# xyfJASON/ctrlora

Hardware: NVIDIA H100
Metric: ddim_steps_per_sec (higher is better)
Workload: dtype fp16 (fp32 accumulate)

## Files before the change

ctrlora_b200/csrc/gemm_sm90.cu:

```cuda
#include "gemm_sm90.cuh"
#include "wgmma.cuh"
#include "ctrlora_b200.h"
#include <stdio.h>
#include <string.h>

namespace ctrl {

__device__ __forceinline__ bool aligned16(const void* ptr) { return (reinterpret_cast<uintptr_t>(ptr) & 15) == 0; }
__device__ __forceinline__ uint32_t pack_h2(float a, float b) {
    __half2 h = __floats2half2_rn(a, b);
    return *reinterpret_cast<uint32_t*>(&h);
}

template <int CW>
__device__ __forceinline__ void epilogue_chunk(const GemmKParams& p, float* v, int c, int bn_out, int n0, bool row_ok,
                                               long long m, int img, int tok) {
    const int nbase = n0 + c;
    const bool full_chunk = (c + CW <= bn_out) && (nbase + CW <= p.N);
    if (!row_ok) return;
    if (p.rowbias) {
        const float* rb = p.rowbias + static_cast<long long>(img) * p.rowbias_ld + nbase;
        if (full_chunk && aligned16(rb)) {
#pragma unroll
            for (int q = 0; q < CW / 4; ++q) {
                const float4 b4 = __ldg(reinterpret_cast<const float4*>(rb) + q);
                v[4 * q] += b4.x; v[4 * q + 1] += b4.y; v[4 * q + 2] += b4.z; v[4 * q + 3] += b4.w;
            }
        } else {
#pragma unroll
            for (int j = 0; j < CW; ++j)
                if (nbase + j < p.N) v[j] += __ldg(rb + j);
        }
    }
    if (p.out_scale != 1.0f) {
#pragma unroll
        for (int j = 0; j < CW; ++j) v[j] *= p.out_scale;
    }
    if (p.residual && p.residual_f32) {
        const float* rp = reinterpret_cast<const float*>(p.residual) + m * p.ldr + nbase;
        if (full_chunk && aligned16(rp)) {
#pragma unroll
            for (int q = 0; q < CW / 4; ++q) {
                const float4 r4 = __ldg(reinterpret_cast<const float4*>(rp) + q);
                v[4 * q] += r4.x; v[4 * q + 1] += r4.y; v[4 * q + 2] += r4.z; v[4 * q + 3] += r4.w;
            }
        } else {
#pragma unroll
            for (int j = 0; j < CW; ++j)
                if (c + j < bn_out && nbase + j < p.N) v[j] += rp[j];
        }
    } else if (p.residual) {
        const __half* rp = p.residual + m * p.ldr + nbase;
        if (full_chunk && aligned16(rp)) {
            uint4 u[CW / 8];
#pragma unroll
            for (int q = 0; q < CW / 8; ++q) u[q] = __ldg(reinterpret_cast<const uint4*>(rp) + q);
#pragma unroll
            for (int q = 0; q < CW / 8; ++q) {
                const __half2* h = reinterpret_cast<const __half2*>(&u[q]);
#pragma unroll
                for (int e = 0; e < 4; ++e) {
                    const float2 f = __half22float2(h[e]);
                    v[q * 8 + e * 2] += f.x;
                    v[q * 8 + e * 2 + 1] += f.y;
                }
            }
        } else {
#pragma unroll
            for (int j = 0; j < CW; ++j)
                if (c + j < bn_out && nbase + j < p.N) v[j] += __half2float(rp[j]);
        }
    }
    int seg = 0, nloc = nbase;
    if (p.seg_width > 0) { seg = nbase / p.seg_width; nloc = nbase - seg * p.seg_width; }
    if (p.transposed[seg]) {
        __half* o = reinterpret_cast<__half*>(p.out[seg]) + (static_cast<long long>(img) * p.seg_width + nloc) * p.tok_pad + tok;
#pragma unroll
        for (int j = 0; j < CW; ++j)
            if (c + j < bn_out && nbase + j < p.N) o[static_cast<long long>(j) * p.tok_pad] = __float2half_rn(v[j]);
        if (p.dup_out) {
            __half* o2 = p.dup_out + m * p.dup_ld + nloc;
#pragma unroll
            for (int j = 0; j < CW; ++j)
                if (c + j < bn_out && nbase + j < p.N) o2[j] = __float2half_rn(v[j]);
        }
    } else if (p.out_f32) {
        float* o = reinterpret_cast<float*>(p.out[seg]) + m * p.ldc + nloc;
        if (full_chunk && aligned16(o)) {
#pragma unroll
            for (int q = 0; q < CW / 4; ++q)
                reinterpret_cast<float4*>(o)[q] = make_float4(v[q * 4], v[q * 4 + 1], v[q * 4 + 2], v[q * 4 + 3]);
        } else {
#pragma unroll
            for (int j = 0; j < CW; ++j)
                if (c + j < bn_out && nbase + j < p.N) o[j] = v[j];
        }
    } else {
        __half* o = reinterpret_cast<__half*>(p.out[seg]) + m * p.ldc + nloc;
        if (full_chunk && aligned16(o)) {
#pragma unroll
            for (int q = 0; q < CW / 8; ++q) {
                uint4 u;
                u.x = pack_h2(v[q * 8 + 0], v[q * 8 + 1]);
                u.y = pack_h2(v[q * 8 + 2], v[q * 8 + 3]);
                u.z = pack_h2(v[q * 8 + 4], v[q * 8 + 5]);
                u.w = pack_h2(v[q * 8 + 6], v[q * 8 + 7]);
                reinterpret_cast<uint4*>(o)[q] = u;
            }
        } else {
#pragma unroll
            for (int j = 0; j < CW; ++j)
                if (c + j < bn_out && nbase + j < p.N) o[j] = __float2half_rn(v[j]);
        }
    }
}

struct GemmUnit {
    int mt, nt, it0, it1, ks, slot;
};
__device__ __forceinline__ GemmUnit gemm_unit(const GemmKParams& p, int u, int m_tiles, int k_iters) {
    GemmUnit w;
    int tile;
    if (u < p.tiles_whole) {
        tile = u;
        w.ks = 0; w.slot = -1; w.it0 = 0; w.it1 = k_iters;
    } else {
        const int v = u - p.tiles_whole;
        w.slot = v / p.splits;
        w.ks = v - w.slot * p.splits;
        tile = p.tiles_whole + w.slot;
        w.it0 = w.ks * p.kiters_per_split;
        w.it1 = min(k_iters, w.it0 + p.kiters_per_split);
    }
    w.mt = tile % m_tiles;
    w.nt = tile / m_tiles;
    return w;
}

__device__ __forceinline__ uint32_t epi_addr(uint32_t base, int r, int col) {
    return base + static_cast<uint32_t>(r * (GEMM_EPI_COLS * 4) + ((((col >> 2) ^ (r & 7)) << 4) | ((col & 3) << 2)));
}

__host__ __device__ constexpr int gemm_slab_cols(int bn_out) { return bn_out % 64 == 0 ? 64 : 32; }
__device__ __forceinline__ uint32_t lds32(uint32_t addr) {
    uint32_t v;
    asm volatile("ld.shared.b32 %0, [%1];" : "=r"(v) : "r"(addr) : "memory");
    return v;
}
__device__ __forceinline__ void sts32(uint32_t addr, uint32_t v) {
    asm volatile("st.shared.b32 [%0], %1;" ::"r"(addr), "r"(v) : "memory");
}
__device__ __forceinline__ float2 h2_to_f2(uint32_t u) { return __half22float2(*reinterpret_cast<const __half2*>(&u)); }

template <bool GEGLU, int BN>
__global__ void __launch_bounds__(GEMM_THREADS, 1)
gemm_wgmma_kernel(const __grid_constant__ CUtensorMap tmA, const __grid_constant__ CUtensorMap tmB,
                  const __grid_constant__ CUtensorMap tmA2, const __grid_constant__ CUtensorMap tmB2,
                  const __grid_constant__ CUtensorMap tmR, const __grid_constant__ CUtensorMap tmO0,
                  const __grid_constant__ CUtensorMap tmO1, const __grid_constant__ CUtensorMap tmO2,
                  const __grid_constant__ GemmKParams p) {
    constexpr int BN_OUT = GEGLU ? BN / 2 : BN;
    constexpr int NACC = BN / 2;
    constexpr int BOX = GEGLU || BN > 256 ? BN / 2 : BN;
    constexpr int SW = gemm_slab_cols(BN_OUT);
    constexpr int NSLAB_TMA = BN_OUT / SW;
    constexpr int SLOT = GEMM_BM * SW * 2;
    extern __shared__ uint8_t smem_raw[];
    uint8_t* smem = reinterpret_cast<uint8_t*>((reinterpret_cast<uintptr_t>(smem_raw) + 1023) & ~uintptr_t(1023));
    uint8_t* ring = smem + p.epi_slots * SLOT;
    uint64_t* bars = reinterpret_cast<uint64_t*>(smem + GEMM_SMEM_DATA);
    uint64_t* full = bars;
    uint64_t* empty = bars + GEMM_MAX_STAGES;
    uint64_t* slot_ready = bars + 2 * GEMM_MAX_STAGES;
    uint64_t* slot_done = slot_ready + GEMM_MAX_SLOTS;
    uint64_t* drained = slot_done + GEMM_MAX_SLOTS;
    volatile int* last_flag = reinterpret_cast<volatile int*>(drained + 1);

    pdl_launch_dependents();
    const int warp = uniform_warp_idx();
    const int lane = threadIdx.x & 31;
    const int nstages = p.stages;
    if (threadIdx.x == 0) {
        tma_prefetch_desc(&tmA);
        tma_prefetch_desc(&tmB);
        if (p.kchunks2 > 0) {
            tma_prefetch_desc(&tmA2);
            tma_prefetch_desc(&tmB2);
        }
        for (int i = 0; i < nstages; ++i) {
            mbar_init(&full[i], 1);
            mbar_init(&empty[i], GEMM_CONSUMERS);
        }
        for (int i = 0; i < p.epi_slots; ++i) {
            mbar_init(&slot_ready[i], 1);
            mbar_init(&slot_done[i], GEMM_CONSUMERS);
        }
        mbar_init(drained, 1);
        fence_barrier_init();
    }
    __syncthreads();
    pdl_wait();

    const int m_tiles = p.tiles_w * p.tiles_h * p.tiles_b;
    const int main_iters = p.taps * p.kchunks;
    const int k_iters = main_iters + p.kchunks2;

    if (warp < 4) {
        setmaxnreg_dec<GEMM_PRODUCER_REGS>();
        if (warp == 0 && elect_one()) {
            const uint32_t tx_bytes = GEMM_A_BYTES + BN * 128;
            int s = 0;
            uint32_t phase = 0;
            for (int u = blockIdx.x; u < p.units; u += gridDim.x) {
                const GemmUnit w = gemm_unit(p, u, m_tiles, k_iters);
                const int tw = w.mt % p.tiles_w, th = (w.mt / p.tiles_w) % p.tiles_h, tb = w.mt / (p.tiles_w * p.tiles_h);
                const int w0 = tw * p.bw - p.pad, h0 = th * p.bh - p.pad, b0 = tb * p.nb, n0 = w.nt * BN_OUT;
                for (int it = w.it0; it < w.it1; ++it) {
                    mbar_wait_nocall(&empty[s], phase ^ 1);
                    uint8_t* dst = ring + s * p.stage_bytes;
                    mbar_expect_tx(&full[s], tx_bytes);
                    if (it < main_iters) {
                        const int tap = it / p.kchunks, kc = it - tap * p.kchunks, ky = tap / p.kw, kx = tap - ky * p.kw;
                        tma_load_4d(dst, &tmA, &full[s], kc * GEMM_BK, w0 + kx, h0 + ky, b0);
                        tma_load_3d(dst + GEMM_A_BYTES, &tmB, &full[s], kc * GEMM_BK, tap, n0);
                        if (BOX < BN)
                            tma_load_3d(dst + GEMM_A_BYTES + BOX * 128, &tmB, &full[s], kc * GEMM_BK, tap, GEGLU ? p.N + n0 : n0 + BOX);
                    } else {
                        const int c0 = (it - main_iters) * GEMM_BK;
                        tma_load_4d(dst, &tmA2, &full[s], c0, w0 + p.pad, h0 + p.pad, b0);
                        tma_load_3d(dst + GEMM_A_BYTES, &tmB2, &full[s], c0, 0, n0);
                        if (BOX < BN) tma_load_3d(dst + GEMM_A_BYTES + BOX * 128, &tmB2, &full[s], c0, 0, n0 + BOX);
                    }
                    if (++s == nstages) { s = 0; phase ^= 1; }
                }
            }
        } else if (warp == 1 && p.tma_tiles > 0 && elect_one()) {
            const int nslots = p.epi_slots;
            auto open = [&](int u, int j, int slot) {
                if (!p.residual) { mbar_arrive(&slot_ready[slot]); return; }
                const int mt = u % m_tiles, nt = u / m_tiles;
                const int tw = mt % p.tiles_w, th = (mt / p.tiles_w) % p.tiles_h, tb = mt / (p.tiles_w * p.tiles_h);
                mbar_expect_tx(&slot_ready[slot], GEMM_BM * SW * 2);
                tma_load_4d(smem + slot * SLOT, &tmR, &slot_ready[slot], nt * BN_OUT + j * SW, tw * p.bw, th * p.bh,
                            tb * p.nb);
            };
            int ou = blockIdx.x, oj = 0;
            for (int k = 0; k < nslots && ou < p.tma_tiles; ++k) {
                open(ou, oj, k);
                if (++oj == NSLAB_TMA) { oj = 0; ou += gridDim.x; }
            }
            int slot = 0, prev_slot = -1;
            uint32_t phase = 0;
            for (int u = blockIdx.x; u < p.tma_tiles; u += gridDim.x) {
                const int mt = u % m_tiles, nt = u / m_tiles;
                const int tw = mt % p.tiles_w, th = (mt / p.tiles_w) % p.tiles_h, tb = mt / (p.tiles_w * p.tiles_h);
                for (int j = 0; j < NSLAB_TMA; ++j) {
                    int col = nt * BN_OUT + j * SW, seg = 0;
                    if (p.seg_width > 0) { seg = col / p.seg_width; col -= seg * p.seg_width; }
                    mbar_wait_nocall(&slot_done[slot], phase);
                    tma_store_4d(seg == 0 ? &tmO0 : seg == 1 ? &tmO1 : &tmO2, smem_u32(smem + slot * SLOT), col,
                                 tw * p.bw, th * p.bh, tb * p.nb);
                    bulk_commit_group();
                    if (prev_slot >= 0) {
                        bulk_wait_group_read<1>();
                        if (ou < p.tma_tiles) {
                            open(ou, oj, prev_slot);
                            if (++oj == NSLAB_TMA) { oj = 0; ou += gridDim.x; }
                        }
                    }
                    prev_slot = slot;
                    if (++slot == nslots) { slot = 0; phase ^= 1; }
                }
            }
            bulk_wait_group<0>();
            mbar_arrive(drained);
        }
        return;
    }

    setmaxnreg_inc<GEMM_CONSUMER_REGS>();
    const int ct = threadIdx.x - 128;
    const int wg = ct >> 7, t = ct & 127;
    const uint32_t ring0 = smem_u32(ring);
    const int fr = ((t >> 5) << 4) + (lane >> 2), cq = 2 * (lane & 3);
    const int er = t & 63, eh = t >> 6;
    const long long slice = static_cast<long long>(GEMM_BM) * BN;
    int s = 0;
    uint32_t phase = 0, slot_pos = 0;
    for (int u = blockIdx.x; u < p.units; u += gridDim.x) {
        const GemmUnit w = gemm_unit(p, u, m_tiles, k_iters);
        float acc[NACC];
#pragma unroll
        for (int i = 0; i < NACC; ++i) acc[i] = 0.f;
        int prev = -1;
        for (int it = w.it0; it < w.it1; ++it) {
            mbar_wait_nocall(&full[s], phase);
            const uint32_t a_base = ring0 + s * p.stage_bytes + wg * 64 * 128;
            const uint32_t b_base = ring0 + s * p.stage_bytes + GEMM_A_BYTES;
            wgmma_fence();
#pragma unroll
            for (int k = 0; k < GEMM_BK / 16; ++k) {
                const uint32_t sc = (it > w.it0 || k > 0) ? 1u : 0u;
                if constexpr (BN > 256) {
                    WgmmaSS<BN / 2, 0, 0>::mma(acc, wgmma_desc_kmajor(a_base + 32 * k), wgmma_desc_kmajor(b_base + 32 * k), sc);
                    WgmmaSS<BN / 2, 0, 0>::mma(acc + NACC / 2, wgmma_desc_kmajor(a_base + 32 * k),
                                               wgmma_desc_kmajor(b_base + (BN / 2) * 128 + 32 * k), sc);
                } else {
                    WgmmaSS<BN, 0, 0>::mma(acc, wgmma_desc_kmajor(a_base + 32 * k), wgmma_desc_kmajor(b_base + 32 * k), sc);
                }
            }
            wgmma_commit();
            wgmma_wait<1>();
            if (prev >= 0) mbar_arrive(&empty[prev]);
            prev = s;
            if (++s == nstages) { s = 0; phase ^= 1; }
        }
        wgmma_wait<0>();
        wgmma_fence_regs<NACC>(acc);
        mbar_arrive(&empty[prev]);

        if (w.slot >= 0) {
            float* frag0 = p.ws + static_cast<long long>(w.slot) * p.splits * slice + ct * 4;
#pragma unroll
            for (int i = 0; i < NACC / 4; ++i)
                __stcg(reinterpret_cast<float4*>(frag0 + w.ks * slice + i * (GEMM_CONSUMERS * 4)),
                       make_float4(acc[4 * i], acc[4 * i + 1], acc[4 * i + 2], acc[4 * i + 3]));
            __threadfence();
            named_bar_sync(1, GEMM_CONSUMERS);
            if (ct == 0) {
                const unsigned int old = atomicAdd(&p.counters[w.slot], 1u);
                const int last = (old == static_cast<unsigned int>(p.splits - 1));
                if (last) p.counters[w.slot] = 0;
                *last_flag = last;
            }
            named_bar_sync(1, GEMM_CONSUMERS);
            if (!*last_flag) continue;
            __threadfence();
#pragma unroll
            for (int i = 0; i < NACC / 4; ++i) {
                float4 t4 = make_float4(0.f, 0.f, 0.f, 0.f);
                for (int sl = 0; sl < p.splits; ++sl) {
                    const float4 x4 = __ldcg(reinterpret_cast<const float4*>(frag0 + sl * slice + i * (GEMM_CONSUMERS * 4)));
                    t4.x += x4.x; t4.y += x4.y; t4.z += x4.z; t4.w += x4.w;
                }
                acc[4 * i] = t4.x; acc[4 * i + 1] = t4.y; acc[4 * i + 2] = t4.z; acc[4 * i + 3] = t4.w;
            }
        }

        const int n0 = w.nt * BN_OUT;
        auto bias_geglu = [&](int i) {
#pragma unroll
            for (int e = 0; e < 2; ++e) {
                const int n = n0 + 8 * i + cq + e;
                float bv = 0.f, bg = 0.f;
                if (p.bias && n < p.N) {
                    bv = __ldg(p.bias + n);
                    if (GEGLU) bg = __ldg(p.bias + p.N + n);
                }
                acc[4 * i + e] += bv;
                acc[4 * i + 2 + e] += bv;
                if (GEGLU) {
                    acc[4 * i + e] *= gelu_erf_f(acc[4 * (i + BN_OUT / 8) + e] + bg);
                    acc[4 * i + 2 + e] *= gelu_erf_f(acc[4 * (i + BN_OUT / 8) + 2 + e] + bg);
                }
            }
        };
        if (GEGLU) {
#pragma unroll
            for (int i = 0; i < BN_OUT / 8; ++i) bias_geglu(i);
        }
        const int tw = w.mt % p.tiles_w, th = (w.mt / p.tiles_w) % p.tiles_h, tb = w.mt / (p.tiles_w * p.tiles_h);
        if (u < p.tma_tiles) {
            const uint32_t row_off = (wg * 64 + fr) * (SW * 2) + cq * 2, row_x = SW == 64 ? (fr & 7) : ((fr >> 1) & 3);
            const float* rb0 = nullptr;
            const float* rb1 = nullptr;
            if (p.rowbias) {
                auto row_img = [&](int r) {
                    const int iw = r % p.bw, ih = (r / p.bw) % p.bh, ib = r / (p.bw * p.bh);
                    const int gw = tw * p.bw + iw, gh = th * p.bh + ih, gb = tb * p.nb + ib;
                    if (gw >= p.W || gh >= p.H || gb >= p.Bn) return 0LL;
                    return ((static_cast<long long>(gb) * p.H + gh) * p.W + gw) / p.rows_per_img;
                };
                rb0 = p.rowbias + row_img(wg * 64 + fr) * p.rowbias_ld;
                rb1 = p.rowbias + row_img(wg * 64 + fr + 8) * p.rowbias_ld;
            }
#pragma unroll
            for (int j = 0; j < NSLAB_TMA; ++j) {
                const int slot = slot_pos & 0xffff;
                mbar_wait_nocall(&slot_ready[slot], slot_pos >> 16);
                const uint32_t sb = ring0 - (p.epi_slots - slot) * SLOT + row_off;
#pragma unroll
                for (int c = 0; c < SW / 8; ++c) {
                    const int i = j * (SW / 8) + c;
                    if (!GEGLU) bias_geglu(i);
                    float v00 = acc[4 * i], v01 = acc[4 * i + 1], v10 = acc[4 * i + 2], v11 = acc[4 * i + 3];
                    const int n = n0 + 8 * i + cq;
                    if (rb0) {
                        if (n < p.N) { v00 = __fadd_rn(v00, __ldg(rb0 + n)); v10 = __fadd_rn(v10, __ldg(rb1 + n)); }
                        if (n + 1 < p.N) { v01 = __fadd_rn(v01, __ldg(rb0 + n + 1)); v11 = __fadd_rn(v11, __ldg(rb1 + n + 1)); }
                    }
                    if (p.out_scale != 1.0f) {
                        v00 = __fmul_rn(v00, p.out_scale); v01 = __fmul_rn(v01, p.out_scale);
                        v10 = __fmul_rn(v10, p.out_scale); v11 = __fmul_rn(v11, p.out_scale);
                    }
                    const uint32_t a0 = sb + ((static_cast<uint32_t>(c) ^ row_x) << 4);
                    const uint32_t a1 = a0 + 8 * SW * 2;
                    if (p.residual) {
                        const float2 r0 = h2_to_f2(lds32(a0)), r1 = h2_to_f2(lds32(a1));
                        v00 = __fadd_rn(v00, r0.x); v01 = __fadd_rn(v01, r0.y);
                        v10 = __fadd_rn(v10, r1.x); v11 = __fadd_rn(v11, r1.y);
                    }
                    sts32(a0, pack_h2(v00, v01));
                    sts32(a1, pack_h2(v10, v11));
                }
                fence_proxy_async_smem();
                mbar_arrive(&slot_done[slot]);
                slot_pos = slot + 1 == p.epi_slots ? (slot_pos & 0x10000) ^ 0x10000 : slot_pos + 1;
            }
            continue;
        }
        if (p.tma_tiles > 0) mbar_wait_nocall(drained, 0);
        const uint32_t stg = ring0 - p.epi_slots * SLOT + wg * (64 * GEMM_EPI_COLS * 4);
        const int r = wg * 64 + er;
        const int iw = r % p.bw, ih = (r / p.bw) % p.bh, ib = r / (p.bw * p.bh);
        const int gw = tw * p.bw + iw, gh = th * p.bh + ih, gb = tb * p.nb + ib;
        const bool row_ok = gw < p.W && gh < p.H && gb < p.Bn;
        const long long m = (static_cast<long long>(gb) * p.H + gh) * p.W + gw;
        const int img = row_ok ? static_cast<int>(m / p.rows_per_img) : 0;
        const int tok = row_ok ? static_cast<int>(m % p.rows_per_img) : 0;
        constexpr int NSLAB = (BN_OUT + GEMM_EPI_COLS - 1) / GEMM_EPI_COLS;
#pragma unroll
        for (int sl = 0; sl < NSLAB; ++sl) {
            const int s0 = sl * GEMM_EPI_COLS;
#pragma unroll
            for (int j = 0; j < GEMM_EPI_COLS / 8; ++j) {
                const int i = sl * (GEMM_EPI_COLS / 8) + j;
                if (i >= BN_OUT / 8) break;
                if (!GEGLU) bias_geglu(i);
                const int col = 8 * j + cq;
                asm volatile("st.shared.v2.f32 [%0], {%1, %2};" ::"r"(epi_addr(stg, fr, col)), "f"(acc[4 * i]), "f"(acc[4 * i + 1])
                             : "memory");
                asm volatile("st.shared.v2.f32 [%0], {%1, %2};" ::"r"(epi_addr(stg, fr + 8, col)), "f"(acc[4 * i + 2]),
                             "f"(acc[4 * i + 3])
                             : "memory");
            }
            named_bar_sync(2 + wg, 128);
            constexpr int CW = BN_OUT > 128 ? 16 : 32;
#pragma unroll
            for (int c1 = 0; c1 < 32; c1 += CW) {
                const int c = s0 + 32 * eh + c1;
                if (c < BN_OUT) {
                    float v[CW];
#pragma unroll
                    for (int q = 0; q < CW / 4; ++q) {
                        const float4 x = lds128f(epi_addr(stg, er, 32 * eh + c1 + 4 * q));
                        v[4 * q] = x.x; v[4 * q + 1] = x.y; v[4 * q + 2] = x.z; v[4 * q + 3] = x.w;
                    }
                    epilogue_chunk<CW>(p, v, c, BN_OUT, n0, row_ok, m, img, tok);
                }
            }
            named_bar_sync(2 + wg, 128);
        }
    }
}

typedef CUresult (*PFN_tmapEncodeTiled)(CUtensorMap*, CUtensorMapDataType, cuuint32_t, void*, const cuuint64_t*,
                                        const cuuint64_t*, const cuuint32_t*, const cuuint32_t*, CUtensorMapInterleave,
                                        CUtensorMapSwizzle, CUtensorMapL2promotion, CUtensorMapFloatOOBfill);

PFN_tmapEncodeTiled get_tmap_encoder() {
    static PFN_tmapEncodeTiled fn = nullptr;
    if (!fn) {
        void* ptr = nullptr;
        cudaDriverEntryPointQueryResult q;
        if (cudaGetDriverEntryPoint("cuTensorMapEncodeTiled", &ptr, cudaEnableDefault, &q) != cudaSuccess ||
            q != cudaDriverEntryPointSuccess)
            return nullptr;
        fn = reinterpret_cast<PFN_tmapEncodeTiled>(ptr);
    }
    return fn;
}

static int make_tmap_f16_sw(CUtensorMap* map, const void* base, int rank, const uint64_t* dims, const uint64_t* strides_bytes,
                            const uint32_t* box, CUtensorMapSwizzle swz);
int make_tmap_f16(CUtensorMap* map, const void* base, int rank, const uint64_t* dims, const uint64_t* strides_bytes,
                  const uint32_t* box) {
    return make_tmap_f16_sw(map, base, rank, dims, strides_bytes, box, CU_TENSOR_MAP_SWIZZLE_128B);
}
static int make_tmap_f16_sw(CUtensorMap* map, const void* base, int rank, const uint64_t* dims, const uint64_t* strides_bytes,
                            const uint32_t* box, CUtensorMapSwizzle swz) {
    PFN_tmapEncodeTiled enc = get_tmap_encoder();
    if (!enc) return CTRLORA_ERR_TMAP;
    cuuint64_t gdim[5], gstr[4];
    cuuint32_t bx[5], es[5];
    for (int i = 0; i < rank; ++i) { gdim[i] = dims[i]; bx[i] = box[i]; es[i] = 1; }
    for (int i = 0; i + 1 < rank; ++i) gstr[i] = strides_bytes[i];
    CUresult r = enc(map, CU_TENSOR_MAP_DATA_TYPE_FLOAT16, rank, const_cast<void*>(base), gdim, gstr, bx, es,
                     CU_TENSOR_MAP_INTERLEAVE_NONE, swz, CU_TENSOR_MAP_L2_PROMOTION_L2_256B,
                     CU_TENSOR_MAP_FLOAT_OOB_FILL_NONE);
    if (r != CUDA_SUCCESS) {
        fprintf(stderr, "ctrlora: cuTensorMapEncodeTiled failed (%d) rank %d dims", (int)r, rank);
        for (int i = 0; i < rank; ++i) fprintf(stderr, " %llu", (unsigned long long)dims[i]);
        fprintf(stderr, " box");
        for (int i = 0; i < rank; ++i) fprintf(stderr, " %u", box[i]);
        fprintf(stderr, "\n");
        return CTRLORA_ERR_TMAP;
    }
    return CTRLORA_OK;
}

static int pow2_floor(int x) {
    int p = 1;
    while (p * 2 <= x) p *= 2;
    return p;
}

static int g_num_sms = 0;
static int g_sm_limit = 0;

int persistent_sms() {
    if (g_num_sms == 0) {
        int dev = 0;
        cudaGetDevice(&dev);
        cudaDeviceGetAttribute(&g_num_sms, cudaDevAttrMultiProcessorCount, dev);
        if (g_num_sms <= 0) return 0;
    }
    return g_sm_limit > 0 && g_sm_limit < g_num_sms ? g_sm_limit : g_num_sms;
}

constexpr double GEMM_L2_BPC = 40.0;
constexpr double GEMM_EPI_FIXED = 600.0;
constexpr double GEMM_EPI_PER_COL = 12.0;
constexpr double GEMM_SPLIT_PER_COL = 12.0;
constexpr int GEMM_MAX_AUTO_SPLIT = 8;
static constexpr int GEMM_WIDE_MIN_KITERS = 40;
static bool g_attr_set = false;

template <bool GEGLU, int BN>
static cudaError_t launch_gemm(dim3 grid, cudaStream_t stream, const CUtensorMap* tm, const GemmKParams& p) {
    return launch_pdl(gemm_wgmma_kernel<GEGLU, BN>, grid, dim3(GEMM_THREADS), (size_t)GEMM_SMEM_BYTES, stream, tm[0], tm[1],
                      tm[2], tm[3], tm[4], tm[5], tm[6], tm[7], p);
}
template <bool GEGLU, int BN>
static bool set_smem_attr() {
    return cudaFuncSetAttribute(gemm_wgmma_kernel<GEGLU, BN>, cudaFuncAttributeMaxDynamicSharedMemorySize, GEMM_SMEM_BYTES) ==
           cudaSuccess;
}

}

using namespace ctrl;

extern "C" int ctrlora_gemm_f16(const ctrlora_gemm_args* a, void* stream_) {
    cudaStream_t stream = reinterpret_cast<cudaStream_t>(stream_);
    if (!a || !a->a || !a->w || !a->out[0]) return CTRLORA_ERR_ARG;
    if (a->a_c % 8 != 0 || a->a_ld % 8 != 0) return CTRLORA_ERR_ARG;
    if (a->kh != a->kw || (a->kh != 1 && a->kh != 3)) return CTRLORA_ERR_UNSUPPORTED;
    if (a->bf16) return CTRLORA_ERR_UNSUPPORTED;
    GemmKParams p;
    memset(&p, 0, sizeof(p));
    p.W = a->a_w; p.H = a->a_h; p.Bn = a->a_b;
    p.bw = pow2_floor(p.W < 128 ? p.W : 128);
    p.bh = pow2_floor(p.H < 128 / p.bw ? p.H : 128 / p.bw);
    p.nb = 128 / (p.bw * p.bh);
    p.tiles_w = (p.W + p.bw - 1) / p.bw;
    p.tiles_h = (p.H + p.bh - 1) / p.bh;
    p.tiles_b = (p.Bn + p.nb - 1) / p.nb;
    p.N = a->n;
    p.taps = a->kh * a->kw; p.kw = a->kw; p.pad = a->pad;
    p.kchunks = (a->a_c + GEMM_BK - 1) / GEMM_BK;
    p.kchunks2 = a->a2 ? (a->a2_c + GEMM_BK - 1) / GEMM_BK : 0;
    p.geglu = a->geglu;
    const int sms = persistent_sms();
    if (sms <= 0) return CTRLORA_ERR_CUDA;
    const int m_tiles = p.tiles_w * p.tiles_h * p.tiles_b;
    const int k_iters = p.taps * p.kchunks + p.kchunks2;
    const bool explicit_split = a->split_k > 0;
    auto plan = [&](int cand, int S, int* s_eff, int* whole) -> double {
        const int bnt = p.geglu ? 2 * cand : cand;
        const long long tiles = (long long)m_tiles * ((p.N + cand - 1) / cand);
        const int kps = (k_iters + S - 1) / S;
        *s_eff = (k_iters + kps - 1) / kps;
        long long w = *s_eff == 1 ? tiles : explicit_split ? 0 : (tiles / sms) * sms;
        const long long tail = tiles - w;
        if (*s_eff > 1 && (!a->splitk_ws || !a->splitk_counters || tail == 0 ||
                           tail * *s_eff * GEMM_BM * bnt * 4 > a->splitk_ws_bytes || tail > a->splitk_counters_len))
            return -1.0;
        *whole = (int)w;
        const double step = fmax(4.0 * bnt, (double)(GEMM_A_BYTES + bnt * 128) / GEMM_L2_BPC);
        const double epi = GEMM_EPI_FIXED + GEMM_EPI_PER_COL * cand;
        const double t_whole = k_iters * step + epi;
        const double t_split = kps * step + epi + GEMM_SPLIT_PER_COL * bnt * (1 + *s_eff);
        return (double)((w + sms - 1) / sms) * t_whole + (double)((tail * *s_eff + sms - 1) / sms) * t_split;
    };
    int bn_out = 0, splits = 1, tiles_whole = 0;
    double best_cost = -1;
    static const int kWidths[] = {GEMM_MAX_BN, 256, 160, 128, 64, 32};
    for (int wi = 0; wi < 6; ++wi) {
        const int cand = p.geglu ? kWidths[wi] / 2 : kWidths[wi];
        if (cand < 32 || (p.geglu && kWidths[wi] == 160)) continue;
        if (a->block_n > 0 && cand != a->block_n) continue;
        if (a->block_n <= 0 && kWidths[wi] > 256 && k_iters < GEMM_WIDE_MIN_KITERS) continue;
        if (a->block_n <= 0 && kWidths[wi] == 160 && k_iters >= GEMM_WIDE_MIN_KITERS) continue;
        if (a->seg_width > 0 && a->seg_width % cand != 0) continue;
        for (int S = explicit_split ? a->split_k : 1; S <= (explicit_split ? a->split_k : GEMM_MAX_AUTO_SPLIT); ++S) {
            int s_eff, whole;
            const double cost = plan(cand, S, &s_eff, &whole);
            if (cost < 0) continue;
            if (best_cost < 0 || cost < best_cost) { best_cost = cost; bn_out = cand; splits = s_eff; tiles_whole = whole; }
        }
    }
    if (bn_out <= 0) {
        return CTRLORA_ERR_ARG;
    }
    p.BN = p.geglu ? 2 * bn_out : bn_out;
    p.n_tiles = (p.N + bn_out - 1) / bn_out;
    p.kiters_per_split = (k_iters + splits - 1) / splits;
    p.splits = (k_iters + p.kiters_per_split - 1) / p.kiters_per_split;
    p.tiles_whole = tiles_whole;
    p.units = tiles_whole + (m_tiles * p.n_tiles - tiles_whole) * p.splits;
    if (p.splits > 1) {
        p.ws = a->splitk_ws;
        p.counters = a->splitk_counters;
    }
    for (int i = 0; i < 3; ++i) { p.out[i] = a->out[i]; p.transposed[i] = a->transposed[i]; }
    const int n_segs = a->seg_width > 0 ? (p.N + a->seg_width - 1) / a->seg_width : 1;
    if (n_segs > 3) return CTRLORA_ERR_ARG;
    auto tma_ok = [](const void* ptr, long long ld) { return (reinterpret_cast<uintptr_t>(ptr) & 15) == 0 && ld % 8 == 0; };
    int tma_segs = 0;
    while (tma_segs < n_segs && !a->transposed[tma_segs]) ++tma_segs;
    bool tma_epi = !a->out_f32 && tma_segs > 0 && (!a->residual || (!a->residual_f32 && tma_ok(a->residual, a->ldr)));
    for (int i = 0; i < n_segs; ++i) {
        if (i < tma_segs ? !a->out[i] || !tma_ok(a->out[i], a->ldc) : !a->transposed[i]) tma_epi = false;
    }
    if (tma_epi) {
        const long long t = tma_segs == n_segs ? (long long)m_tiles * p.n_tiles : (long long)m_tiles * tma_segs * (a->seg_width / bn_out);
        p.tma_tiles = (int)(t < tiles_whole ? t : tiles_whole);
    }
    const int slab_cols = gemm_slab_cols(bn_out);
    const int slot_bytes = GEMM_BM * slab_cols * 2;
    int epi_want = p.tma_tiles > 0 ? (bn_out / slab_cols) * slot_bytes : GEMM_EPI_BYTES;
    if (epi_want < GEMM_EPI_BYTES) epi_want = GEMM_EPI_BYTES;
    p.stage_bytes = GEMM_A_BYTES + ((p.BN * 128 + 1023) / 1024) * 1024;
    p.stages = (GEMM_SMEM_DATA - epi_want) / p.stage_bytes;
    if (p.stages < 3) p.stages = 3;
    if (p.stages > GEMM_MAX_STAGES) p.stages = GEMM_MAX_STAGES;
    p.epi_slots = (GEMM_SMEM_DATA - p.stages * p.stage_bytes) / slot_bytes;
    if (p.epi_slots > GEMM_MAX_SLOTS) p.epi_slots = GEMM_MAX_SLOTS;
    p.seg_width = a->seg_width;
    p.ldc = a->ldc; p.out_f32 = a->out_f32;
    p.bias = a->bias; p.rowbias = a->rowbias;
    p.rows_per_img = a->rows_per_img > 0 ? a->rows_per_img : p.W * p.H;
    p.residual = reinterpret_cast<const __half*>(a->residual); p.ldr = a->ldr;
    p.residual_f32 = a->residual_f32;
    p.rowbias_ld = a->rowbias_ld > 0 ? a->rowbias_ld : a->n;
    p.out_scale = a->out_scale;
    p.head_dim = a->head_dim; p.tok_pad = a->tok_pad;
    p.dup_out = reinterpret_cast<__half*>(a->dup_out); p.dup_ld = a->dup_ld;

    const int b_box = p.geglu || p.BN > 256 ? p.BN / 2 : p.BN;
    CUtensorMap tm[8];
    CUtensorMap &tmA = tm[0], &tmB = tm[1], &tmA2 = tm[2], &tmB2 = tm[3];
    {
        uint64_t dims[4] = {(uint64_t)a->a_c, (uint64_t)p.W, (uint64_t)p.H, (uint64_t)p.Bn};
        uint64_t str[3] = {(uint64_t)a->a_ld * 2, (uint64_t)a->a_ld * 2 * p.W, (uint64_t)a->a_ld * 2 * p.W * p.H};
        uint32_t box[4] = {GEMM_BK, (uint32_t)p.bw, (uint32_t)p.bh, (uint32_t)p.nb};
        int rc = make_tmap_f16(&tmA, a->a, 4, dims, str, box);
        if (rc) return rc;
        const uint64_t rows = p.geglu ? 2ull * p.N : (uint64_t)p.N;
        uint64_t wd[3] = {(uint64_t)a->a_c, (uint64_t)p.taps, rows};
        uint64_t ws[2] = {(uint64_t)a->a_c * 2, (uint64_t)a->a_c * 2 * p.taps};
        uint32_t wb[3] = {GEMM_BK, 1, (uint32_t)b_box};
        rc = make_tmap_f16(&tmB, a->w, 3, wd, ws, wb);
        if (rc) return rc;
    }
    if (a->a2) {
        if (!a->w2 || a->a2_c % 8 != 0 || a->a2_ld % 8 != 0 || p.geglu) return CTRLORA_ERR_ARG;
        uint64_t dims[4] = {(uint64_t)a->a2_c, (uint64_t)p.W, (uint64_t)p.H, (uint64_t)p.Bn};
        uint64_t str[3] = {(uint64_t)a->a2_ld * 2, (uint64_t)a->a2_ld * 2 * p.W, (uint64_t)a->a2_ld * 2 * p.W * p.H};
        uint32_t box[4] = {GEMM_BK, (uint32_t)p.bw, (uint32_t)p.bh, (uint32_t)p.nb};
        int rc = make_tmap_f16(&tmA2, a->a2, 4, dims, str, box);
        if (rc) return rc;
        uint64_t wd[3] = {(uint64_t)a->a2_c, 1, (uint64_t)p.N};
        uint64_t ws[2] = {(uint64_t)a->a2_c * 2, (uint64_t)a->a2_c * 2};
        uint32_t wb[3] = {GEMM_BK, 1, (uint32_t)b_box};
        rc = make_tmap_f16(&tmB2, a->w2, 3, wd, ws, wb);
        if (rc) return rc;
    } else {
        tmA2 = tmA;
        tmB2 = tmB;
    }
    for (int i = 4; i < 8; ++i) tm[i] = tmA;
    if (p.tma_tiles > 0) {
        const CUtensorMapSwizzle swz = slab_cols == 64 ? CU_TENSOR_MAP_SWIZZLE_128B : CU_TENSOR_MAP_SWIZZLE_64B;
        const uint32_t box[4] = {(uint32_t)slab_cols, (uint32_t)p.bw, (uint32_t)p.bh, (uint32_t)p.nb};
        auto pixel_map = [&](CUtensorMap* m, const void* base, int cols, long long ld) {
            uint64_t dims[4] = {(uint64_t)cols, (uint64_t)p.W, (uint64_t)p.H, (uint64_t)p.Bn};
            uint64_t str[3] = {(uint64_t)ld * 2, (uint64_t)ld * 2 * p.W, (uint64_t)ld * 2 * p.W * p.H};
            return make_tmap_f16_sw(m, base, 4, dims, str, box, swz);
        };
        if (a->residual) {
            int rc = pixel_map(&tm[4], a->residual, p.N, a->ldr);
            if (rc) return rc;
        }
        for (int i = 0; i < tma_segs; ++i) {
            const int cols = a->seg_width > 0 ? (p.N - i * a->seg_width < a->seg_width ? p.N - i * a->seg_width : a->seg_width) : p.N;
            int rc = pixel_map(&tm[5 + i], a->out[i], cols, a->ldc);
            if (rc) return rc;
        }
    }
    if (!g_attr_set) {
        if (!set_smem_attr<false, 32>() || !set_smem_attr<false, 64>() || !set_smem_attr<false, 128>() ||
            !set_smem_attr<false, 160>() || !set_smem_attr<false, 256>() || !set_smem_attr<false, 320>() || !set_smem_attr<true, 64>() ||
            !set_smem_attr<true, 128>() || !set_smem_attr<true, 256>() || !set_smem_attr<true, 320>())
            return CTRLORA_ERR_CUDA;
        g_attr_set = true;
    }
    const dim3 grid((unsigned)(p.units < sms ? p.units : sms));
    cudaError_t lrc;
    if (p.geglu) lrc = p.BN == 64  ? launch_gemm<true, 64>(grid, stream, tm, p)
                     : p.BN == 128 ? launch_gemm<true, 128>(grid, stream, tm, p)
                     : p.BN == 256 ? launch_gemm<true, 256>(grid, stream, tm, p)
                                   : launch_gemm<true, 320>(grid, stream, tm, p);
    else lrc = p.BN == 32  ? launch_gemm<false, 32>(grid, stream, tm, p)
             : p.BN == 64  ? launch_gemm<false, 64>(grid, stream, tm, p)
             : p.BN == 128 ? launch_gemm<false, 128>(grid, stream, tm, p)
             : p.BN == 160 ? launch_gemm<false, 160>(grid, stream, tm, p)
             : p.BN == 256 ? launch_gemm<false, 256>(grid, stream, tm, p)
                           : launch_gemm<false, 320>(grid, stream, tm, p);
    if (lrc != cudaSuccess) return CTRLORA_ERR_CUDA;
    return cudaGetLastError() == cudaSuccess ? CTRLORA_OK : CTRLORA_ERR_CUDA;
}

extern "C" int ctrlora_set_sm_limit(int limit) {
    if (limit < 0) return CTRLORA_ERR_ARG;
    g_sm_limit = limit;
    return CTRLORA_OK;
}
```

Measured before the change: 34.78.

## Add ping-pong consumer schedule for short-K GEMMs with TMA epilogue

Adds a ping-pong variant of the persistent WGMMA GEMM. The two consumer warpgroups take alternating whole tiles and hand off through named barriers, so one group's epilogue overlaps the other's mainloop. The host planner gets a cost model for this mode and picks it for short-K, non-split, full-TMA-epilogue cases. It adds new template instantiations and a more complex barrier protocol, and it risks higher register pressure because each thread now holds BN accumulators.

```diff
diff --git a/ctrlora_b200/csrc/gemm_sm90.cu b/ctrlora_b200/csrc/gemm_sm90.cu
--- a/ctrlora_b200/csrc/gemm_sm90.cu
+++ b/ctrlora_b200/csrc/gemm_sm90.cu
@@ -152,7 +152,143 @@
 }
 __device__ __forceinline__ float2 h2_to_f2(uint32_t u) { return __half22float2(*reinterpret_cast<const __half2*>(&u)); }
 
+struct RingPos {
+    int slot;
+    uint32_t phase;
+};
+__host__ __device__ __forceinline__ RingPos ring_pos(uint32_t idx, int n) {
+    return RingPos{static_cast<int>(idx % static_cast<uint32_t>(n)), (idx / static_cast<uint32_t>(n)) & 1u};
+}
+
 template <bool GEGLU, int BN>
+__device__ __forceinline__ void gemm_pingpong_consumers(const GemmKParams& p, uint8_t* ring, uint64_t* full,
+                                                        uint64_t* empty, uint64_t* slot_ready, uint64_t* slot_done,
+                                                        int m_tiles, int k_iters) {
+    constexpr int BN_OUT = GEGLU ? BN / 2 : BN;
+    constexpr int HALF = BN / 2;
+    constexpr int SW = gemm_slab_cols(BN_OUT);
+    constexpr int NSLAB_TMA = BN_OUT / SW;
+    constexpr int SLOT = GEMM_BM * SW * 2;
+    static_assert(BN <= 160, "ping-pong tiles hold BN accumulators per thread");
+    const int ct = threadIdx.x - 128;
+    const int wg = ct >> 7, t = ct & 127, lane = threadIdx.x & 31;
+    const uint32_t ring0 = smem_u32(ring);
+    const int fr = ((t >> 5) << 4) + (lane >> 2), cq = 2 * (lane & 3);
+    const int n_local = (p.units - static_cast<int>(blockIdx.x) + static_cast<int>(gridDim.x) - 1) / static_cast<int>(gridDim.x);
+    for (int q = wg; q < n_local; q += 2) {
+        const int u = blockIdx.x + q * gridDim.x;
+        const int mt = u % m_tiles, nt = u / m_tiles;
+        float acc[BN];
+#pragma unroll
+        for (int i = 0; i < BN; ++i) acc[i] = 0.f;
+        if (q > 0) named_bar_sync(4 + wg, 256);
+        RingPos rp = ring_pos(static_cast<uint32_t>(q) * k_iters, p.stages);
+        int s = rp.slot, prev = -1;
+        uint32_t phase = rp.phase;
+        for (int it = 0; it < k_iters; ++it) {
+            mbar_wait_nocall(&full[s], phase);
+            const uint32_t a_base = ring0 + s * p.stage_bytes;
+            const uint32_t b_base = a_base + GEMM_A_BYTES;
+            wgmma_fence();
+#pragma unroll
+            for (int k = 0; k < GEMM_BK / 16; ++k) {
+                const uint32_t sc = (it > 0 || k > 0) ? 1u : 0u;
+                const uint64_t db = wgmma_desc_kmajor(b_base + 32 * k);
+                WgmmaSS<BN, 0, 0>::mma(acc, wgmma_desc_kmajor(a_base + 32 * k), db, sc);
+                WgmmaSS<BN, 0, 0>::mma(acc + HALF, wgmma_desc_kmajor(a_base + 64 * 128 + 32 * k), db, sc);
+            }
+            wgmma_commit();
+            wgmma_wait<1>();
+            if (prev >= 0) mbar_arrive(&empty[prev]);
+            prev = s;
+            if (++s == p.stages) { s = 0; phase ^= 1; }
+        }
+        if (q + 1 < n_local) named_bar_arrive(4 + (wg ^ 1), 256);
+        wgmma_wait<0>();
+        wgmma_fence_regs<BN>(acc);
+        mbar_arrive(&empty[prev]);
+
+        const int n0 = nt * BN_OUT;
+        auto bias_geglu = [&](float* a, int i) {
+#pragma unroll
+            for (int e = 0; e < 2; ++e) {
+                const int n = n0 + 8 * i + cq + e;
+                float bv = 0.f, bg = 0.f;
+                if (p.bias && n < p.N) {
+                    bv = __ldg(p.bias + n);
+                    if (GEGLU) bg = __ldg(p.bias + p.N + n);
+                }
+                a[4 * i + e] += bv;
+                a[4 * i + 2 + e] += bv;
+                if (GEGLU) {
+                    a[4 * i + e] *= gelu_erf_f(a[4 * (i + BN_OUT / 8) + e] + bg);
+                    a[4 * i + 2 + e] *= gelu_erf_f(a[4 * (i + BN_OUT / 8) + 2 + e] + bg);
+                }
+            }
+        };
+        if (GEGLU) {
+#pragma unroll
+            for (int h = 0; h < 2; ++h)
+#pragma unroll
+                for (int i = 0; i < BN_OUT / 8; ++i) bias_geglu(acc + h * HALF, i);
+        }
+        const int tw = mt % p.tiles_w, th = (mt / p.tiles_w) % p.tiles_h, tb = mt / (p.tiles_w * p.tiles_h);
+        const uint32_t row_x = SW == 64 ? (fr & 7) : ((fr >> 1) & 3);
+        const float* rb[4] = {nullptr, nullptr, nullptr, nullptr};
+        if (p.rowbias) {
+            auto row_img = [&](int r) {
+                const int iw = r % p.bw, ih = (r / p.bw) % p.bh, ib = r / (p.bw * p.bh);
+                const int gw = tw * p.bw + iw, gh = th * p.bh + ih, gb = tb * p.nb + ib;
+                if (gw >= p.W || gh >= p.H || gb >= p.Bn) return 0LL;
+                return ((static_cast<long long>(gb) * p.H + gh) * p.W + gw) / p.rows_per_img;
+            };
+#pragma unroll
+            for (int r = 0; r < 4; ++r) rb[r] = p.rowbias + row_img((r >> 1) * 64 + fr + (r & 1) * 8) * p.rowbias_ld;
+        }
+#pragma unroll
+        for (int j = 0; j < NSLAB_TMA; ++j) {
+            const uint32_t idx = static_cast<uint32_t>(q) * NSLAB_TMA + j;
+            const RingPos sp = ring_pos(idx, p.epi_slots);
+            if (idx >= static_cast<uint32_t>(p.epi_slots)) mbar_wait_nocall(&slot_done[sp.slot], sp.phase ^ 1);
+            mbar_wait_nocall(&slot_ready[sp.slot], sp.phase);
+#pragma unroll
+            for (int h = 0; h < 2; ++h) {
+                float* a = acc + h * HALF;
+                const uint32_t sb = ring0 - (p.epi_slots - sp.slot) * SLOT + (h * 64 + fr) * (SW * 2) + cq * 2;
+#pragma unroll
+                for (int c = 0; c < SW / 8; ++c) {
+                    const int i = j * (SW / 8) + c;
+                    if (!GEGLU) bias_geglu(a, i);
+                    float v00 = a[4 * i], v01 = a[4 * i + 1], v10 = a[4 * i + 2], v11 = a[4 * i + 3];
+                    const int n = n0 + 8 * i + cq;
+                    if (rb[0]) {
+                        const float* r0 = rb[2 * h];
+                        const float* r1 = rb[2 * h + 1];
+                        if (n < p.N) { v00 = __fadd_rn(v00, __ldg(r0 + n)); v10 = __fadd_rn(v10, __ldg(r1 + n)); }
+                        if (n + 1 < p.N) { v01 = __fadd_rn(v01, __ldg(r0 + n + 1)); v11 = __fadd_rn(v11, __ldg(r1 + n + 1)); }
+                    }
+                    if (p.out_scale != 1.0f) {
+                        v00 = __fmul_rn(v00, p.out_scale); v01 = __fmul_rn(v01, p.out_scale);
+                        v10 = __fmul_rn(v10, p.out_scale); v11 = __fmul_rn(v11, p.out_scale);
+                    }
+                    const uint32_t a0 = sb + ((static_cast<uint32_t>(c) ^ row_x) << 4);
+                    const uint32_t a1 = a0 + 8 * SW * 2;
+                    if (p.residual) {
+                        const float2 r0 = h2_to_f2(lds32(a0)), r1 = h2_to_f2(lds32(a1));
+                        v00 = __fadd_rn(v00, r0.x); v01 = __fadd_rn(v01, r0.y);
+                        v10 = __fadd_rn(v10, r1.x); v11 = __fadd_rn(v11, r1.y);
+                    }
+                    sts32(a0, pack_h2(v00, v01));
+                    sts32(a1, pack_h2(v10, v11));
+                }
+            }
+            fence_proxy_async_smem();
+            mbar_arrive(&slot_done[sp.slot]);
+        }
+    }
+}
+
+template <bool GEGLU, int BN, bool PP>
 __global__ void __launch_bounds__(GEMM_THREADS, 1)
 gemm_wgmma_kernel(const __grid_constant__ CUtensorMap tmA, const __grid_constant__ CUtensorMap tmB,
                   const __grid_constant__ CUtensorMap tmA2, const __grid_constant__ CUtensorMap tmB2,
@@ -189,11 +325,11 @@
         }
         for (int i = 0; i < nstages; ++i) {
             mbar_init(&full[i], 1);
-            mbar_init(&empty[i], GEMM_CONSUMERS);
+            mbar_init(&empty[i], PP ? 128 : GEMM_CONSUMERS);
         }
         for (int i = 0; i < p.epi_slots; ++i) {
             mbar_init(&slot_ready[i], 1);
-            mbar_init(&slot_done[i], GEMM_CONSUMERS);
+            mbar_init(&slot_done[i], PP ? 128 : GEMM_CONSUMERS);
         }
         mbar_init(drained, 1);
         fence_barrier_init();
@@ -279,6 +415,10 @@
     }
 
     setmaxnreg_inc<GEMM_CONSUMER_REGS>();
+    if constexpr (PP) {
+        gemm_pingpong_consumers<GEGLU, BN>(p, ring, full, empty, slot_ready, slot_done, m_tiles, k_iters);
+        return;
+    }
     const int ct = threadIdx.x - 128;
     const int wg = ct >> 7, t = ct & 127;
     const uint32_t ring0 = smem_u32(ring);
@@ -534,16 +674,17 @@
 constexpr double GEMM_SPLIT_PER_COL = 12.0;
 constexpr int GEMM_MAX_AUTO_SPLIT = 8;
 static constexpr int GEMM_WIDE_MIN_KITERS = 40;
+static constexpr int GEMM_PP_MAX_KITERS = GEMM_WIDE_MIN_KITERS;
 static bool g_attr_set = false;
 
-template <bool GEGLU, int BN>
+template <bool GEGLU, int BN, bool PP = false>
 static cudaError_t launch_gemm(dim3 grid, cudaStream_t stream, const CUtensorMap* tm, const GemmKParams& p) {
-    return launch_pdl(gemm_wgmma_kernel<GEGLU, BN>, grid, dim3(GEMM_THREADS), (size_t)GEMM_SMEM_BYTES, stream, tm[0], tm[1],
+    return launch_pdl(gemm_wgmma_kernel<GEGLU, BN, PP>, grid, dim3(GEMM_THREADS), (size_t)GEMM_SMEM_BYTES, stream, tm[0], tm[1],
                       tm[2], tm[3], tm[4], tm[5], tm[6], tm[7], p);
 }
-template <bool GEGLU, int BN>
+template <bool GEGLU, int BN, bool PP = false>
 static bool set_smem_attr() {
-    return cudaFuncSetAttribute(gemm_wgmma_kernel<GEGLU, BN>, cudaFuncAttributeMaxDynamicSharedMemorySize, GEMM_SMEM_BYTES) ==
+    return cudaFuncSetAttribute(gemm_wgmma_kernel<GEGLU, BN, PP>, cudaFuncAttributeMaxDynamicSharedMemorySize, GEMM_SMEM_BYTES) ==
            cudaSuccess;
 }
 
@@ -574,8 +715,18 @@
     const int sms = persistent_sms();
     if (sms <= 0) return CTRLORA_ERR_CUDA;
     const int m_tiles = p.tiles_w * p.tiles_h * p.tiles_b;
+    const int n_segs = a->seg_width > 0 ? (p.N + a->seg_width - 1) / a->seg_width : 1;
+    if (n_segs > 3) return CTRLORA_ERR_ARG;
+    auto tma_ok = [](const void* ptr, long long ld) { return (reinterpret_cast<uintptr_t>(ptr) & 15) == 0 && ld % 8 == 0; };
+    int tma_segs = 0;
+    while (tma_segs < n_segs && !a->transposed[tma_segs]) ++tma_segs;
+    bool tma_epi = !a->out_f32 && tma_segs > 0 && (!a->residual || (!a->residual_f32 && tma_ok(a->residual, a->ldr)));
+    for (int i = 0; i < n_segs; ++i) {
+        if (i < tma_segs ? !a->out[i] || !tma_ok(a->out[i], a->ldc) : !a->transposed[i]) tma_epi = false;
+    }
     const int k_iters = p.taps * p.kchunks + p.kchunks2;
     const bool explicit_split = a->split_k > 0;
+    const bool pp_launch = tma_epi && tma_segs == n_segs && k_iters < GEMM_PP_MAX_KITERS && a->split_k <= 1;
     auto plan = [&](int cand, int S, int* s_eff, int* whole) -> double {
         const int bnt = p.geglu ? 2 * cand : cand;
         const long long tiles = (long long)m_tiles * ((p.N + cand - 1) / cand);
@@ -593,7 +744,15 @@
         const double t_split = kps * step + epi + GEMM_SPLIT_PER_COL * bnt * (1 + *s_eff);
         return (double)((w + sms - 1) / sms) * t_whole + (double)((tail * *s_eff + sms - 1) / sms) * t_split;
     };
+    auto plan_pp = [&](int cand) -> double {
+        const int bnt = p.geglu ? 2 * cand : cand;
+        const long long per_cta = ((long long)m_tiles * ((p.N + cand - 1) / cand) + sms - 1) / sms;
+        const double step = fmax(4.0 * bnt, (double)(GEMM_A_BYTES + bnt * 128) / GEMM_L2_BPC);
+        const double epi = GEMM_EPI_FIXED + 2.0 * GEMM_EPI_PER_COL * cand;
+        return (double)per_cta * fmax(k_iters * step, epi) + epi;
+    };
     int bn_out = 0, splits = 1, tiles_whole = 0;
+    bool pingpong = false;
     double best_cost = -1;
     static const int kWidths[] = {GEMM_MAX_BN, 256, 160, 128, 64, 32};
     for (int wi = 0; wi < 6; ++wi) {
@@ -603,11 +762,22 @@
         if (a->block_n <= 0 && kWidths[wi] > 256 && k_iters < GEMM_WIDE_MIN_KITERS) continue;
         if (a->block_n <= 0 && kWidths[wi] == 160 && k_iters >= GEMM_WIDE_MIN_KITERS) continue;
         if (a->seg_width > 0 && a->seg_width % cand != 0) continue;
+        const bool pp_width = pp_launch && (p.geglu ? cand == 64 : cand >= 64 && cand <= 160);
+        if (pp_width) {
+            const double cost = plan_pp(cand);
+            if (best_cost < 0 || cost < best_cost || a->block_n > 0) {
+                best_cost = cost; bn_out = cand; splits = 1; pingpong = true;
+                tiles_whole = m_tiles * ((p.N + cand - 1) / cand);
+            }
+            if (a->block_n > 0) break;
+        }
         for (int S = explicit_split ? a->split_k : 1; S <= (explicit_split ? a->split_k : GEMM_MAX_AUTO_SPLIT); ++S) {
             int s_eff, whole;
             const double cost = plan(cand, S, &s_eff, &whole);
             if (cost < 0) continue;
-            if (best_cost < 0 || cost < best_cost) { best_cost = cost; bn_out = cand; splits = s_eff; tiles_whole = whole; }
+            if (best_cost < 0 || cost < best_cost) {
+                best_cost = cost; bn_out = cand; splits = s_eff; tiles_whole = whole; pingpong = false;
+            }
         }
     }
     if (bn_out <= 0) {
@@ -624,15 +794,6 @@
         p.counters = a->splitk_counters;
     }
     for (int i = 0; i < 3; ++i) { p.out[i] = a->out[i]; p.transposed[i] = a->transposed[i]; }
-    const int n_segs = a->seg_width > 0 ? (p.N + a->seg_width - 1) / a->seg_width : 1;
-    if (n_segs > 3) return CTRLORA_ERR_ARG;
-    auto tma_ok = [](const void* ptr, long long ld) { return (reinterpret_cast<uintptr_t>(ptr) & 15) == 0 && ld % 8 == 0; };
-    int tma_segs = 0;
-    while (tma_segs < n_segs && !a->transposed[tma_segs]) ++tma_segs;
-    bool tma_epi = !a->out_f32 && tma_segs > 0 && (!a->residual || (!a->residual_f32 && tma_ok(a->residual, a->ldr)));
-    for (int i = 0; i < n_segs; ++i) {
-        if (i < tma_segs ? !a->out[i] || !tma_ok(a->out[i], a->ldc) : !a->transposed[i]) tma_epi = false;
-    }
     if (tma_epi) {
         const long long t = tma_segs == n_segs ? (long long)m_tiles * p.n_tiles : (long long)m_tiles * tma_segs * (a->seg_width / bn_out);
         p.tma_tiles = (int)(t < tiles_whole ? t : tiles_whole);
@@ -712,13 +873,22 @@
     if (!g_attr_set) {
         if (!set_smem_attr<false, 32>() || !set_smem_attr<false, 64>() || !set_smem_attr<false, 128>() ||
             !set_smem_attr<false, 160>() || !set_smem_attr<false, 256>() || !set_smem_attr<false, 320>() || !set_smem_attr<true, 64>() ||
-            !set_smem_attr<true, 128>() || !set_smem_attr<true, 256>() || !set_smem_attr<true, 320>())
+            !set_smem_attr<true, 128>() || !set_smem_attr<true, 256>() || !set_smem_attr<true, 320>() ||
+            !set_smem_attr<false, 64, true>() || !set_smem_attr<false, 128, true>() || !set_smem_attr<false, 160, true>() ||
+            !set_smem_attr<true, 128, true>())
             return CTRLORA_ERR_CUDA;
         g_attr_set = true;
     }
     const dim3 grid((unsigned)(p.units < sms ? p.units : sms));
     cudaError_t lrc;
-    if (p.geglu) lrc = p.BN == 64  ? launch_gemm<true, 64>(grid, stream, tm, p)
+    if (pingpong) {
+        if (p.tma_tiles != p.units || p.splits != 1 || p.epi_slots < 2 || p.epi_slots < bn_out / slab_cols)
+            return CTRLORA_ERR_ARG;
+        lrc = p.geglu      ? launch_gemm<true, 128, true>(grid, stream, tm, p)
+            : p.BN == 64  ? launch_gemm<false, 64, true>(grid, stream, tm, p)
+            : p.BN == 128 ? launch_gemm<false, 128, true>(grid, stream, tm, p)
+                          : launch_gemm<false, 160, true>(grid, stream, tm, p);
+    } else if (p.geglu) lrc = p.BN == 64  ? launch_gemm<true, 64>(grid, stream, tm, p)
                      : p.BN == 128 ? launch_gemm<true, 128>(grid, stream, tm, p)
                      : p.BN == 256 ? launch_gemm<true, 256>(grid, stream, tm, p)
                                    : launch_gemm<true, 320>(grid, stream, tm, p);
```

New measurement: 35.96 (median of 6 runs). +3.4%, better.
